# pd3/bcftools

Measured on AMD Instinct MI355X. Metric: variant sites/sec (mpileup|call -m), 1000-sample 30x WGS synthetic, higher is better.
Workload: dtype u8/i32 + f64 likelihood sums

## Files before the change

bcftools_amd/csrc/glfgen.hip:

```cpp
#include <hip/hip_runtime.h>
#include <cstdlib>
#include "kernels.h"

namespace bcfgpu {

#define WG 256
#ifndef GLF_WAVES
#define GLF_WAVES 5
#endif
#define DEF_MAPQ 20
#define CAP_DIST 25

#define NT16_INT_TBL 0x4444444344424104ull
__device__ __forceinline__ int nt16_int(int c) { return (int)((NT16_INT_TBL >> (4 * (c & 15))) & 7); }
__device__ __forceinline__ int tri(int j, int k) { return k * (k + 1) / 2 + j; }

__device__ __forceinline__ uint32_t wave_sum_u32(uint32_t v)
{
    #pragma unroll
    for (int o = 32; o > 0; o >>= 1) v += __shfl_xor(v, o);
    return v;
}

#define LDS_FK   0
#define LDS_CNT  2112
#ifndef NRANK
#define NRANK 10
#endif
#define NSLOT    NRANK
#ifndef FU
#define FU       4
#endif
#define LDS_HIST_OFF (LDS_CNT + NSLOT * WG * 4)
#define HP_SIZE 280
#define HP_MQS  220
#define NPART 17
static_assert(NPART == SITE_NSUM + 3, "phase A's partial sums: the site totals and three mapQ >= 59 counts");

#define KEY_PACK(rev, q, b, sc) ((uint32_t)(rev) | (uint32_t)(q) << 1 | (uint32_t)(b) << 7 | (uint32_t)(sc) << 10)
#define KEY_REV(k)  ((k) & 1u)
#define KEY_Q(k)    (((k) >> 1) & 63u)
#define KEY_B(k)    (((k) >> 7) & 7u)
#define KEY_SC(k)   (((k) >> 10) & 1u)
#define KEY_PRIM    0x800u

#ifndef WR
#define WR 2
#endif
struct PrimSrc {
    const uint16_t *kpp;
    __device__ __forceinline__ uint32_t key(int j) const { return kpp[j]; }
    __device__ __forceinline__ bool ok(uint32_t k) const { return k != 0; }
    __device__ __forceinline__ int operator()(int j) const { const uint32_t k = key(j); return ok(k) ? (int)(k & 0x7f) : -1; }
};
struct BaseSrc {
    const uint16_t *kp; int b;
    __device__ __forceinline__ uint32_t key(int i) const { return kp[i]; }
    __device__ __forceinline__ bool ok(uint32_t k) const { return KEY_B(k) == (uint32_t)b; }
    __device__ __forceinline__ int operator()(int i) const { const uint32_t k = key(i); return ok(k) ? (int)(k & 0x7f) : -1; }
};
__device__ __forceinline__ uint32_t popc64(uint64_t x) { return (uint32_t)__popc((uint32_t)x) + (uint32_t)__popc((uint32_t)(x >> 32)); }
template <bool FIRST, bool CHK, class Src>
__device__ __forceinline__ void count_keys(uint32_t *s_slot, uint64_t qm, int tid, Src src, int nsrc)
{
    const uint64_t qm1 = qm >> 1;
    for (int j = 0; __any(j < nsrc); j += FU) {
        if (j < nsrc) {
            uint32_t k4[FU];
            #pragma unroll
            for (int u = 0; u < FU; ++u) k4[u] = src.key(j + u);
            #pragma unroll
            for (int u = 0; u < FU; ++u) {
                const uint32_t k = k4[u], q = KEY_Q(k);
                const uint32_t r = popc64(qm1 >> q);
                bool take = src.ok(k) && (u == 0 || j + u < nsrc);
                if (!FIRST) take = take && ((qm >> q) & 1ull);
                if (CHK) take = take && r < (uint32_t)NRANK;
                const uint32_t rv = (uint32_t)((int32_t)(k << 31) >> 31);
                if (take) atomicAdd(&s_slot[r * WG + tid], (rv & 1u) | (~rv & 0x100u));
            }
        }
    }
}
template <bool FIRST, class Src>
__device__ __forceinline__ uint32_t count_runs(uint32_t *s_slot, uint64_t qm, int tid, Src src, int nsrc)
{
    #pragma unroll
    for (int k = 0; k < NRANK; ++k) s_slot[k * WG + tid] = 0;
    if (__any(popc64(qm) > (uint32_t)NRANK)) count_keys<FIRST, true>(s_slot, qm, tid, src, nsrc);
    else count_keys<FIRST, false>(s_slot, qm, tid, src, nsrc);
    uint32_t qs = 0;
    uint64_t m = qm;
    #pragma unroll
    for (int r = 0; r < NRANK && __any(m != 0); ++r) {
        if (m != 0) {
            const uint32_t q = 63u - (uint32_t)__builtin_clzll(m);
            const uint32_t c = s_slot[r * WG + tid];
            s_slot[r * WG + tid] = c | q << 16;
            qs = __builtin_amdgcn_udot4(c, q | q << 8, qs, false);
            m &= ~(1ull << q);
        }
    }
    return qs;
}

template <class Src>
__device__ __forceinline__ double walk_runs(uint32_t *s_slot, uint64_t qm, const double *s_fk, const char *bbase, int tid,
                                            uint32_t brow, Src src, int nsrc, uint32_t &rev_out, uint32_t &qs_out)
{
    double bs = 0;
    uint32_t qs = 0;
    uint32_t wpack = 0;
    uint32_t cnt = 0;
    uint32_t koff = brow;
    uint32_t qoff = 0;
    uint32_t r = 0;
    uint32_t d_nx = 0;
    auto slot_of = [&](uint32_t rk) -> uint32_t { return s_slot[min(rk, (uint32_t)NRANK - 1u) * WG + tid]; };
    auto step = [&](uint32_t (&off)[WR], uint32_t (&wi)[WR]) -> bool {
        const bool pop = cnt == 0 && r < NRANK;
        cnt = pop ? (d_nx & 0xffu) | (d_nx & 0xff00u) << 8 : cnt;
        qoff = pop ? (d_nx & 0x3f0000u) << 3 : qoff;
        r += pop ? 1u : 0u;
        d_nx = slot_of(r);
        const uint32_t sh = (cnt & 0xffffu) ? 0u : 16u;
        const uint32_t left = (cnt >> sh) & 0xffffu;
        const uint32_t w = (wpack >> sh) & 0xffffu;
        const uint32_t o1 = qoff + koff;
        #pragma unroll
        for (uint32_t u = 0; u < WR; ++u) {
            const bool act = left > u;
            wi[u] = act ? w + u : 256u;
            off[u] = act ? o1 + (u << 11) : brow;
        }
        const uint32_t took = min(left, (uint32_t)WR);
        wpack += took << sh; cnt -= took << sh;
        koff += took << 11;
        return __any(left != 0);
    };
    #define WALK_LOAD(B, F, off_, wi_) do { _Pragma("unroll") for (int u_ = 0; u_ < WR; ++u_) { \
        B[u_] = *reinterpret_cast<const double*>(bbase + (off_)[u_]); F[u_] = s_fk[(wi_)[u_]]; } } while (0)
    #define WALK_ADD(B, F) do { _Pragma("unroll") for (int u_ = 0; u_ < WR; ++u_) bs += F[u_] * B[u_]; } while (0)
    bool first = true;
    while (__any(qm != 0)) {
        qs += first ? count_runs<true>(s_slot, qm, tid, src, nsrc) : count_runs<false>(s_slot, qm, tid, src, nsrc);
        first = false; r = 0;
        d_nx = slot_of(0);
        double bx[WR], fx[WR], by[WR], fy[WR];
        uint32_t off[WR], wi[WR];
        bool ax = step(off, wi);
        WALK_LOAD(bx, fx, off, wi);
        bool ay = step(off, wi);
        WALK_LOAD(by, fy, off, wi);
        while (ax) {
            WALK_ADD(bx, fx);
            ax = step(off, wi);
            WALK_LOAD(bx, fx, off, wi);
            if (!ay) break;
            WALK_ADD(by, fy);
            ay = step(off, wi);
            WALK_LOAD(by, fy, off, wi);
        }
        WALK_ADD(bx, fx);
        WALK_ADD(by, fy);
        if (__any(__popcll(qm) > NRANK)) {
            uint64_t m = qm;
            for (int k = 0; k < NRANK && m; ++k) m &= ~(1ull << (63 - __clzll((long long)m)));
            qm = m;
        } else qm = 0;
    }
    #undef WALK_ADD
    #undef WALK_LOAD
    rev_out = wpack & 0xffffu; qs_out = qs;
    return bs;
}

struct ReadSums {
    uint32_t t_bq, t_bq2, t_mq, t_mq2, t_md, t_md2;
    uint32_t d_bq, d_bq2, d_mq, d_mq2, d_md, d_md2;
    __device__ __forceinline__ void clear() { t_bq = t_bq2 = t_mq = t_mq2 = t_md = t_md2 = d_bq = d_bq2 = d_mq = d_mq2 = d_md = d_md2 = 0; }
};
struct ReadCounts {
    uint32_t ori, mq0, m59, ref59, rev59;
    __device__ __forceinline__ void clear() { ori = mq0 = m59 = ref59 = rev59 = 0; }
};
typedef unsigned short v2u16 __attribute__((ext_vector_type(2)));

__device__ __forceinline__ uint32_t perm(uint32_t hi, uint32_t lo, uint32_t sel) { return __builtin_amdgcn_perm(hi, lo, sel); }
#define SEL_EVEN 0x0c020c00u
#define SEL_ODD  0x0c030c01u
#define SEL_JOIN 0x06020400u
#define SEL_GE8  0x07030501u
__device__ __forceinline__ v2u16 as_v2(uint32_t x) { return __builtin_bit_cast(v2u16, x); }
__device__ __forceinline__ uint32_t as_u(v2u16 x) { return __builtin_bit_cast(uint32_t, x); }
__device__ __forceinline__ uint32_t pk_min(uint32_t a, uint32_t b) { return as_u(__builtin_elementwise_min(as_v2(a), as_v2(b))); }
__device__ __forceinline__ uint32_t pk_max(uint32_t a, uint32_t b) { return as_u(__builtin_elementwise_max(as_v2(a), as_v2(b))); }
__device__ __forceinline__ uint32_t nonzero80(uint32_t x) { return (((x & 0x7f7f7f7fu) + 0x7f7f7f7fu) | x) & 0x80808080u; }
__device__ __forceinline__ uint32_t bytes_of80(uint32_t m) { return m | (m - (m >> 7)); }
__device__ __forceinline__ uint32_t byte_at(uint32_t x, int u) { return (x >> (8 * u)) & 0xffu; }

template <bool INDEL, bool LDS_HIST, bool DEEP>
__global__ __launch_bounds__(WG) __attribute__((amdgpu_waves_per_eu(GLF_WAVES, GLF_WAVES))) void glfgen_kernel(const GlfgenParams P)
{
    extern __shared__ __align__(16) unsigned char smem[];
    if (DEEP && (blockIdx.x >= P.deep_ctr[0] || P.deep_list[2 * blockIdx.x] == 0xffffffffu)) return;
    const int cap = DEEP ? 0x7ffffff0 : P.lds_cap;
    double   *s_fk  = reinterpret_cast<double*>(smem + LDS_FK);
    uint32_t *s_cnt = reinterpret_cast<uint32_t*>(smem + LDS_CNT);
    int      *s_hist = reinterpret_cast<int*>(smem + LDS_HIST_OFF);
    unsigned long long *s_tot = reinterpret_cast<unsigned long long*>(s_hist + (size_t)P.hist_slots * HP_SIZE);
    uint32_t *s_part = s_cnt;
    const int pcol = P.part_cols;
    uint16_t *s_key = DEEP ? P.deep_keys + P.deep_list[2 * blockIdx.x + 1]
                           : reinterpret_cast<uint16_t*>(s_tot + (size_t)P.hist_slots * SITE_NSUM);
    __shared__ unsigned int s_next, s_skip;

    const int tid = threadIdx.x;
    const int S = P.n_smpl;
    const long ncells = (long)P.n_sites * S;
    const long cell0 = DEEP ? (long)P.deep_list[2 * blockIdx.x] : (long)blockIdx.x * WG;
    const long cell_end = DEEP ? cell0 + 1 : min(cell0 + WG, ncells);
    const int site0 = (int)(cell0 / S);
    const int site_last = (int)((cell_end - 1) / S);

    const long cell = cell0 + tid;
    const bool active = cell < cell_end;

    s_fk[tid] = P.fk[tid];
    if (tid < 8) s_fk[256 + tid] = 0.0;
    if (LDS_HIST) {
        for (int i = tid; i < P.hist_slots * HP_SIZE; i += WG) s_hist[i] = 0;
        for (int i = tid; i < P.hist_slots * SITE_NSUM; i += WG) s_tot[i] = 0;
    }

    int site = 0, ref4c = 4;
    uint32_t beg = 0, end = 0;
    if (active) {
        site = (int)(cell / S);
        beg = P.off[cell]; end = P.off[cell + 1];
        if (!INDEL) ref4c = nt16_int(P.ref16[site]);
    }
    const int primary = INDEL ? 0 : ref4c;
    uint32_t fmt_flag = (uint32_t)P.fmt_flag;
    asm volatile("" : "+s"(fmt_flag));
    const bool want_epos = (fmt_flag & (BCFGPU_INFO_RPB | BCFGPU_INFO_VDB)) != 0;
    const bool want_scr = (fmt_flag & (BCFGPU_INFO_SCR | BCFGPU_FMT_SCR)) != 0;
    const uint32_t span_end = P.off[cell_end];
    uint32_t n_reads_tot = P.n_reads, min_baseQ = (uint32_t)P.min_baseQ, capQ = (uint32_t)P.capQ;
    asm volatile("" : "+s"(n_reads_tot), "+s"(min_baseQ), "+s"(capQ));
    const uint32_t *p_rd = P.rd, *p_aux = P.aux, *p_off = P.off;
    const uint8_t *p_epos = P.epos;
    asm volatile("" : "+s"(p_rd), "+s"(p_aux), "+s"(p_off), "+s"(p_epos));

    bool done = !active;
    bool deep = false;
    if (!DEEP && active && end - beg > (uint32_t)cap - 3u) {
        deep = true;
        const uint32_t need = (end - beg + 16u) & ~7u;
        const uint32_t slot = atomicAdd(&P.deep_ctr[0], 1u), at = atomicAdd(&P.deep_ctr[1], need);
        const bool room = at + need <= P.deep_key_cap;
        if (slot < P.deep_cap) { P.deep_list[2 * slot] = room ? (uint32_t)cell : 0xffffffffu; P.deep_list[2 * slot + 1] = room ? at : 0u; }
        if (slot >= P.deep_cap || !room) { atomicExch(P.err, BCFGPU_E_DEPTH); atomicExch(&P.deep_ctr[2], 1u); }
    }
    uint32_t base = p_off[cell0];

    for (;;) {
        const uint32_t abase = base & ~3u;
        const uint32_t lim = DEEP ? span_end : min(abase + (uint32_t)cap, span_end);
        if (tid == 0) { s_next = 0xffffffffu; s_skip = 0; }
        if (LDS_HIST) {
            int i0 = tid;
            asm volatile("" : "+v"(i0));
            for (int i = i0; i < P.hist_slots * NPART * pcol; i += WG) s_part[i] = 0;
        }
        __syncthreads();
        const bool cand = !done && !deep && beg >= base && end <= lim;
        if (!done && !cand) atomicMin(&s_next, beg);
        __syncthreads();
        const uint32_t nb = s_next;
        const uint32_t rlim = min(nb, lim);
        const bool part = cand && end <= rlim;

        for (int sg = site0; sg <= site_last; ++sg) {
            const long c_lo = max(cell0, (long)sg * S), c_hi = min(cell_end, (long)(sg + 1) * S);
            const uint32_t rb = max(p_off[c_lo], base), re = min(p_off[c_hi], rlim);
            if (rb >= re) continue;
            const int ref_base = INDEL ? -1 : (int)P.ref16[sg];
            const uint32_t ref4 = INDEL ? 4u : (uint32_t)nt16_int(ref_base);
            const uint32_t primq = INDEL ? 0u : ref4;
            const unsigned long long tbl = (NT16_INT_TBL & ~0xfull) | (unsigned long long)ref4;
            int *hist = LDS_HIST ? s_hist + (sg - site0) * HP_SIZE : P.hist + (long)sg * H_SIZE;
            ReadSums A; A.clear();
            ReadCounts C; C.clear();
            const uint32_t tlo_lo = 0x04010000u | ref4, tlo_hi = 0x04040402u, thi_lo = 0x04040403u, thi_hi = 0x04040404u;
            const uint32_t kq = 0x01000100u - min(min_baseQ, 256u) * 0x00010001u;
            const uint32_t cap2 = min(capQ, 0xffffu) * 0x00010001u;
            const uint32_t refb4 = (uint32_t)(ref_base & 15) * 0x01010101u, prim4 = primq * 0x01010101u;
            const uint32_t scm = want_scr ? 0x04040404u : 0u;
            const bool all_diff = !INDEL && ref4 >= 4;
            const bool no_ref = INDEL || ref_base < 0 || ref_base > 15;

            auto quad = [&](const uint4 &w4, const uint4 &a4, uint32_t e4, uint32_t vm4, uint32_t &k01, uint32_t &k23) {
                const uint32_t t0 = perm(w4.y, w4.x, 0x05010400u), t1 = perm(w4.y, w4.x, 0x07030602u);
                const uint32_t t2 = perm(w4.w, w4.z, 0x05010400u), t3 = perm(w4.w, w4.z, 0x07030602u);
                uint32_t B4 = perm(t2, t0, 0x05040100u);
                const uint32_t M4 = perm(t2, t0, 0x07060302u);
                const uint32_t F4 = (vm4 & perm(t3, t1, 0x05040100u)) | (~vm4 & 0x80808080u);
                const uint32_t D4 = perm(t3, t1, 0x07060302u);
                uint32_t QR4, BB4;
                uint32_t ok80;
                const uint32_t seen80 = (INDEL ? F4 : F4 | F4 << 1) & 0x80808080u ^ 0x80808080u;
                if (INDEL) {
                    uint32_t qv[4], bv[4];
                    const uint32_t av[4] = { a4.x, a4.y, a4.z, a4.w }, wv[4] = { w4.x, w4.y, w4.z, w4.w };
                    #pragma unroll
                    for (int u = 0; u < 4; ++u) {
                        const uint32_t ax = av[u];
                        uint32_t b = (ax >> 16) & 0xf, q = ax & 0xff;
                        if (q < min_baseQ) { b = 0; q = wv[u] & 0xff; }
                        bv[u] = min(b, 4u);
                        qv[u] = min(q, (ax >> 8) & 0xff);
                    }
                    B4 = perm(perm(a4.w, a4.z, 0x04000c0cu), perm(a4.y, a4.x, 0x0c0c0400u), 0x07060100u);
                    QR4 = qv[0] | qv[1] << 8 | qv[2] << 16 | qv[3] << 24;
                    BB4 = bv[0] | bv[1] << 8 | bv[2] << 16 | bv[3] << 24;
                    ok80 = seen80;
                } else {
                    const uint32_t ge = perm(perm(0, B4, SEL_ODD) + kq, perm(0, B4, SEL_EVEN) + kq, SEL_GE8);
                    ok80 = seen80 & ge << 7;
                    QR4 = B4;
                    const uint32_t s = F4 & 0x07070707u;
                    BB4 = perm(perm(thi_hi, thi_lo, s), perm(tlo_hi, tlo_lo, s), 0x03020100u | (F4 >> 1 & 0x04040404u));
                }
                const uint32_t OK4 = bytes_of80(ok80);
                const uint32_t me = perm(0, M4, SEL_EVEN), mo = perm(0, M4, SEL_ODD);
                const uint32_t mfe = pk_min(me + (uint32_t)__mul24((int)perm(0, me + 0x00010001u, SEL_ODD), DEF_MAPQ - 255), cap2);
                const uint32_t mfo = pk_min(mo + (uint32_t)__mul24((int)perm(0, mo + 0x00010001u, SEL_ODD), DEF_MAPQ - 255), cap2);
                const uint32_t qe = pk_max(pk_min(pk_min(perm(0, QR4, SEL_EVEN), mfe), 0x003f003fu), 0x00040004u);
                const uint32_t qo = pk_max(pk_min(pk_min(perm(0, QR4, SEL_ODD), mfo), 0x003f003fu), 0x00040004u);
                const uint32_t Q4 = perm(qo, qe, SEL_JOIN);
                const uint32_t Mf4 = perm(mfo, mfe, SEL_JOIN);
                const uint32_t Df4 = perm(pk_min(perm(0, D4, SEL_ODD), 0x00190019u), pk_min(perm(0, D4, SEL_EVEN), 0x00190019u), SEL_JOIN);
                const uint32_t m59_80 = ok80 & perm(mfo + 0x00c500c5u, mfe + 0x00c500c5u, SEL_GE8) << 7;
                const uint32_t nref80 = no_ref ? 0x80808080u : nonzero80((F4 ^ refb4) & 0x0f0f0f0fu);
                C.ori += __builtin_popcount(seen80);
                C.mq0 += __builtin_popcount(ok80 & ~nonzero80(M4));
                C.m59 += __builtin_popcount(m59_80);
                C.ref59 += __builtin_popcount(m59_80 & ~nref80);
                C.rev59 += __builtin_popcount(m59_80 & F4 << 3);
                const uint32_t nprim80 = nonzero80(BB4 ^ prim4);
                const uint32_t klo = (((F4 >> 4) & 0x01010101u) | Q4 << 1 | (BB4 & 0x01010101u) << 7) & OK4;
                const uint32_t khi = (((BB4 >> 1) & 0x03030303u) | ((F4 >> 3) & scm) | ((nprim80 ^ 0x80808080u) >> 4)) & OK4;
                k01 = perm(khi, klo, 0x05010400u); k23 = perm(khi, klo, 0x07030602u);
                const uint32_t Bm = B4 & OK4, Mm = Mf4 & OK4, Dm = Df4 & OK4;
                A.t_bq = __builtin_amdgcn_udot4(Bm, 0x01010101u, A.t_bq, false); A.t_bq2 = __builtin_amdgcn_udot4(Bm, Bm, A.t_bq2, false);
                A.t_mq = __builtin_amdgcn_udot4(Mm, 0x01010101u, A.t_mq, false); A.t_mq2 = __builtin_amdgcn_udot4(Mm, Mm, A.t_mq2, false);
                A.t_md = __builtin_amdgcn_udot4(Dm, 0x01010101u, A.t_md, false); A.t_md2 = __builtin_amdgcn_udot4(Dm, Dm, A.t_md2, false);
                const uint32_t dif80 = ok80 & (all_diff ? 0x80808080u : nprim80);
                if (dif80) {
                    const uint32_t DM = bytes_of80(dif80);
                    const uint32_t bd = Bm & DM, qd = Mm & DM, dd = Dm & DM;
                    A.d_bq = __builtin_amdgcn_udot4(bd, 0x01010101u, A.d_bq, false); A.d_bq2 = __builtin_amdgcn_udot4(bd, bd, A.d_bq2, false);
                    A.d_mq = __builtin_amdgcn_udot4(qd, 0x01010101u, A.d_mq, false); A.d_mq2 = __builtin_amdgcn_udot4(qd, qd, A.d_mq2, false);
                    A.d_md = __builtin_amdgcn_udot4(dd, 0x01010101u, A.d_md, false); A.d_md2 = __builtin_amdgcn_udot4(dd, dd, A.d_md2, false);
                }
                #pragma unroll
                for (int u = 0; u < 4; ++u) {
                    if (!((ok80 >> (8 * u + 7)) & 1)) continue;
                    const bool isref = !((nref80 >> (8 * u + 7)) & 1), rev = (F4 >> (8 * u + 4)) & 1;
                    const uint32_t bq = byte_at(B4, u), mapQ = byte_at(Mf4, u), pos = byte_at(e4, u);
                    const bool m59 = (m59_80 >> (8 * u + 7)) & 1;
                    if (LDS_HIST) {
                        const int inc = isref ? 1 : 0x10000;
                        atomicAdd(&hist[H_REF_POS + pos], inc);
                        atomicAdd(&hist[H_REF_BQ + min(bq, 59u)], inc);
                        if (!m59) {
                            atomicAdd(&hist[H_REF_MQ + mapQ], inc);
                            atomicAdd(&hist[HP_MQS + mapQ], rev ? 0x10000 : 1);
                        }
                    } else {
                        const uint32_t aoff = isref ? 0u : (uint32_t)H_ALT_OFF;
                        atomicAdd(&hist[aoff + H_REF_POS + pos], 1);
                        atomicAdd(&hist[aoff + H_REF_BQ + min(bq, 59u)], 1);
                        if (!m59) {
                            atomicAdd(&hist[aoff + H_REF_MQ + mapQ], 1);
                            atomicAdd(&hist[(rev ? H_REV_MQS : H_FWD_MQS) + mapQ], 1);
                        }
                    }
                }
            };

            const uint32_t g0 = rb & ~3u;
            uint4 w4n = make_uint4(0, 0, 0, 0), a4n = make_uint4(0, 0, 0, 0);
            uint32_t e4n = 0;
            auto fetch = [&](uint32_t i4) {
                if (i4 >= re) return;
                if (i4 + 3 < n_reads_tot) {
                    w4n = *reinterpret_cast<const uint4*>(p_rd + i4);
                    if (want_epos) e4n = *reinterpret_cast<const uint32_t*>(p_epos + i4);
                    if (INDEL) a4n = *reinterpret_cast<const uint4*>(p_aux + i4);
                } else {
                    uint32_t t4[4] = {0, 0, 0, 0}, x4[4] = {0, 0, 0, 0};
                    e4n = 0;
                    for (int j = 0; j < 4; ++j) if (i4 + j < n_reads_tot) {
                        t4[j] = p_rd[i4 + j];
                        if (want_epos) e4n |= (uint32_t)p_epos[i4 + j] << (8 * j);
                        if (INDEL) x4[j] = p_aux[i4 + j];
                    }
                    w4n = make_uint4(t4[0], t4[1], t4[2], t4[3]); a4n = make_uint4(x4[0], x4[1], x4[2], x4[3]);
                }
            };
            fetch(g0 + 4u * tid);
            for (uint32_t i4 = g0 + 4u * tid; i4 < re; i4 += 4u * WG) {
                const uint4 w4 = w4n, a4 = a4n;
                const uint32_t e4 = e4n;
                fetch(i4 + 4u * WG);
                const uint32_t lo = rb > i4 ? rb - i4 : 0u, hi = min(re - i4, 4u);
                const uint32_t vm4 = (0xffffffffu << (8 * lo)) & (hi == 4u ? 0xffffffffu : ~(0xffffffffu << (8 * hi)));
                uint32_t k01, k23;
                quad(w4, a4, e4, vm4, k01, k23);
                const uint32_t ko = i4 - abase;
                if (vm4 == 0xffffffffu) {
                    *reinterpret_cast<uint2*>(s_key + ko) = make_uint2(k01, k23);
                } else {
                    const uint32_t kv[4] = { k01 & 0xffffu, k01 >> 16, k23 & 0xffffu, k23 >> 16 };
                    #pragma unroll
                    for (int u = 0; u < 4; ++u) if ((vm4 >> (8 * u)) & 1) s_key[ko + u] = (uint16_t)kv[u];
                }
            }
            const uint32_t v[NPART] = { A.t_bq - A.d_bq, A.t_bq2 - A.d_bq2, A.d_bq, A.d_bq2, A.t_mq - A.d_mq, A.t_mq2 - A.d_mq2, A.d_mq, A.d_mq2,
                                        A.t_md - A.d_md, A.t_md2 - A.d_md2, A.d_md, A.d_md2, C.ori, C.mq0, C.m59, C.ref59, C.rev59 };
            if (LDS_HIST) {
                uint32_t *pt = s_part + (sg - site0) * (NPART * pcol) + (tid & (pcol - 1));
                #pragma unroll
                for (int j = 0; j < NPART; ++j) atomicAdd(&pt[j * pcol], v[j]);
            } else {
                unsigned long long *tot = P.site_sums + (size_t)sg * SITE_NSUM;
                uint32_t x[NPART];
                #pragma unroll
                for (int j = 0; j < NPART; ++j) x[j] = wave_sum_u32(v[j]);
                if ((tid & 63) == 0) {
                    #pragma unroll
                    for (int j = 0; j < SITE_NSUM; ++j) if (x[j]) atomicAdd(&tot[j], (unsigned long long)x[j]);
                    const uint32_t m59 = x[SITE_NSUM], ref59 = x[SITE_NSUM + 1], rev59 = x[SITE_NSUM + 2];
                    if (ref59) atomicAdd(&hist[H_REF_MQ + 59], (int)ref59);
                    if (m59 - ref59) atomicAdd(&hist[H_ALT_MQ + 59], (int)(m59 - ref59));
                    if (m59 - rev59) atomicAdd(&hist[H_FWD_MQS + 59], (int)(m59 - rev59));
                    if (rev59) atomicAdd(&hist[H_REV_MQS + 59], (int)rev59);
                }
            }
        }
        __syncthreads();
        if (LDS_HIST) {
            const int nslot = min(P.hist_slots, P.n_sites - site0), q4 = pcol >> 2;
            for (int i = tid; i < nslot * NPART * 4; i += WG) {
                const uint32_t *pt = s_part + (i >> 2) * pcol + (i & 3) * q4;
                unsigned long long x = 0;
                for (int k = 0; k < q4; ++k) x += pt[k];
                x += __shfl_xor(x, 1); x += __shfl_xor(x, 2);
                if ((i & 3) == 0 && x) {
                    const int vi = i >> 2, sl = vi / NPART, j = vi % NPART;
                    if (j < SITE_NSUM) s_tot[sl * SITE_NSUM + j] += x;
                    else {
                        const uint32_t c = (uint32_t)x;
                        int *h = s_hist + sl * HP_SIZE;
                        if (j == SITE_NSUM) { atomicAdd(&h[H_REF_MQ + 59], (int)(c << 16)); atomicAdd(&h[HP_MQS + 59], (int)c); }
                        else if (j == SITE_NSUM + 1) atomicAdd(&h[H_REF_MQ + 59], (int)(c - (c << 16)));
                        else atomicAdd(&h[HP_MQS + 59], (int)((c << 16) - c));
                    }
                }
            }
            __syncthreads();
        }

        uint16_t *kp_w = s_key + (part ? beg - abase : 0);
        const uint16_t *kp = kp_w;
        const int cnt_raw = part ? (int)(end - beg) : 0;
        if (__any(cnt_raw > BCFGPU_MAX_DEPTH)) {
            if (cnt_raw > BCFGPU_MAX_DEPTH) {
                uint32_t nus = 0;
                for (int i = 0; i < cnt_raw; ++i) nus += kp_w[i] != 0 ? 1u : 0u;
                const volatile unsigned long long *t = reinterpret_cast<const volatile unsigned long long*>(P.crp);
                uint64_t *qs64_p = reinterpret_cast<uint64_t*>(t[2]); uint32_t *misc_p = reinterpret_cast<uint32_t*>(t[6]);
                uint32_t mark = 0;
                if (nus > BCFGPU_MAX_DEPTH) {
                    uint32_t qs[4] = {0, 0, 0, 0}, af[4] = {0, 0, 0, 0}, ar[4] = {0, 0, 0, 0}, cn[4] = {0, 0, 0, 0}, sc = 0, acc = 0;
                    const bool all_diff = !INDEL && ref4c >= 4;
                    bool planned = false;
                    if (P.draw_bits) {
                        uint32_t nm = 0;
                        for (int i = 0; i < cnt_raw; ++i) { const uint32_t ri = beg + (uint32_t)i; nm += (kp_w[i] != 0 && ((P.draw_bits[ri >> 5] >> (ri & 31)) & 1u)) ? 1u : 0u; }
                        planned = nm == BCFGPU_MAX_DEPTH;
                    }
                    for (int i = 0; i < cnt_raw; ++i) {
                        const uint32_t k = kp_w[i];
                        if (k == 0) continue;
                        const uint32_t rev = KEY_REV(k), q = KEY_Q(k), b = KEY_B(k);
                        const uint32_t dr = ((all_diff || !(k & KEY_PRIM)) ? 2u : 0u) | rev;
                        #pragma unroll
                        for (uint32_t x = 0; x < 4; ++x) {
                            qs[x] += b == x ? q : 0u;
                            af[x] += (b == x && !rev) ? 1u : 0u; ar[x] += (b == x && rev) ? 1u : 0u;
                            cn[x] += dr == x ? 1u : 0u;
                        }
                        sc += KEY_SC(k);
                        bool stays = ++acc <= BCFGPU_MAX_DEPTH;
                        if (planned) { const uint32_t ri = beg + (uint32_t)i; stays = ((P.draw_bits[ri >> 5] >> (ri & 31)) & 1u) != 0; }
                        if (!stays) kp_w[i] = 0;
                    }
                    const uint32_t slot = atomicAdd(P.wide_ctr, 1u);
                    const uint32_t big = af[0] | af[1] | af[2] | af[3] | ar[0] | ar[1] | ar[2] | ar[3] | cn[0] | cn[1] | cn[2] | cn[3] | sc;
                    if (slot >= P.wide_cap || big > 0xffffu) atomicExch(P.err, BCFGPU_E_DEPTH);
                    else {
                        WideRec *w = reinterpret_cast<WideRec*>(t[7]) + slot;
                        #pragma unroll
                        for (int x = 0; x < 4; ++x) { w->qs[x] = qs[x]; w->ad[x] = af[x] | ar[x] << 16; }
                        w->cnt[0] = cn[0] | cn[1] << 16; w->cnt[1] = cn[2] | cn[3] << 16;
                        w->scr = sc; w->n = nus; w->cell = (uint32_t)cell; w->pad[0] = w->pad[1] = w->pad[2] = 0;
                        qs64_p[cell] = WIDE_QS_MARK | slot;
                        mark = CR_WIDE;
                    }
                    if (!planned) atomicAdd(P.trunc, 1u);
                }
                misc_p[cell] = mark;
            }
        }
        uint32_t scr = 0;
        if (want_scr) for (int i = 0; i < cnt_raw; ++i) scr += KEY_SC((uint32_t)kp[i]);
        uint64_t qmask = 0;
        uint32_t n_prim = 0;
        uint64_t qs64 = 0;
        uint64_t ad64 = 0;
        uint32_t n_b4 = 0;
        uint32_t o_rev = 0, n_other = 0;
        {
            uint32_t k_nx = kp[0];
            for (int i = 0; i < cnt_raw; ++i) {
                const uint32_t k = k_nx;
                k_nx = kp[i + 1];
                const uint32_t pb = k >> 11;
                qmask |= (uint64_t)pb << KEY_Q(k);
                n_prim += pb;
                if (k - 1u < KEY_PRIM - 1u) {
                    const uint32_t t = kp_w[n_other], rev = KEY_REV(k), q = KEY_Q(k), b = KEY_B(k);
                    kp_w[n_other] = (uint16_t)k; kp_w[i] = (uint16_t)t;
                    ++n_other; o_rev += rev;
                    if (b < 4) { qs64 += (uint64_t)q << (16 * b); ad64 += 1ull << (8 * b + 32 * rev); }
                    else ++n_b4;
                }
            }
        }
        const uint32_t n = n_prim + n_other;
        const bool dead_cell = n == 0;
        const char *bbase = reinterpret_cast<const char*>(P.beta);
        const uint32_t brow = n << 3;

        double bsum[5] = {0, 0, 0, 0, 0};
        uint32_t prim_rev = 0, qs_prim = 0;
        {
            const uint16_t *kpp = kp + n_other;
            const PrimSrc psrc{kpp};
            const double bs = walk_runs(s_cnt, qmask, s_fk, bbase, tid, brow, psrc, dead_cell ? 0 : cnt_raw - (int)n_other, prim_rev, qs_prim);
            #pragma unroll
            for (int b = 0; b < 5; ++b) if (b == primary) bsum[b] = bs;
        }
        if (primary < 4) {
            qs64 += (uint64_t)qs_prim << (16 * primary);
            ad64 += (uint64_t)(n_prim - prim_rev) << (8 * primary) | (uint64_t)prim_rev << (8 * primary + 32);
        } else n_b4 += n_prim;
        int c[5];
        #pragma unroll
        for (int b = 0; b < 4; ++b) c[b] = (int)((ad64 >> (8 * b)) & 0xff) + (int)((ad64 >> (8 * b + 32)) & 0xff);
        c[4] = (int)n_b4;
        if (__any(n_other > 0)) {
            #pragma unroll 1
            for (int b = 0; b < 5; ++b) {
                int cb = b == 0 ? c[0] : b == 1 ? c[1] : b == 2 ? c[2] : b == 3 ? c[3] : c[4];
                if (b == primary || dead_cell) cb = 0;
                if (!__any(cb > 0)) continue;
                const BaseSrc src{kp, b};
                const int no = cb > 0 ? (int)n_other : 0;
                double bs;
                if (!__any(cb > 1)) {
                    int key = -1;
                    for (int i = 0; __any(i < no); ++i) { const int k7 = i < no ? src(i) : -1; if (k7 >= 0) key = k7; }
                    const uint32_t off1 = key >= 0 ? ((uint32_t)(key >> 1) << 19) + brow : brow;
                    const double B1 = *reinterpret_cast<const double*>(bbase + off1);
                    const double F1 = key >= 0 ? s_fk[0] : s_fk[256];
                    bs = 0.;
                    bs += F1 * B1;
                } else {
                uint64_t qm = 0;
                for (int i = 0; i < no; ++i) { const int key = src(i); if (key >= 0) qm |= 1ull << (key >> 1); }
                uint32_t r_, q_;
                bs = walk_runs(s_cnt, qm, s_fk, bbase, tid, brow, src, no, r_, q_);
                }
                if (cb > 0) {
                    #pragma unroll
                    for (int bb = 0; bb < 5; ++bb) if (bb == b) bsum[bb] = bs;
                }
            }
        }
        const uint32_t n_rev = prim_rev + o_rev;

        uint32_t code = 0;
        CallretPlanes cr;
        {
            const volatile unsigned long long *t = reinterpret_cast<const volatile unsigned long long*>(P.crp);
            cr.p15 = reinterpret_cast<float*>(t[0]); cr.pa = reinterpret_cast<float*>(t[1]);
            cr.qs64 = reinterpret_cast<uint64_t*>(t[2]); cr.adf = reinterpret_cast<uint32_t*>(t[3]);
            cr.adr = reinterpret_cast<uint32_t*>(t[4]); cr.cnt4 = reinterpret_cast<uint32_t*>(t[5]);
            cr.misc = reinterpret_cast<uint32_t*>(t[6]);
        }
        if (part) {
            const int nbases = (c[0] > 0) + (c[1] > 0) + (c[2] > 0) + (c[3] > 0) + (c[4] > 0);
            if (nbases <= 1) {
                const int b = c[1] > 0 ? 1 : c[2] > 0 ? 2 : c[3] > 0 ? 3 : c[4] > 0 ? 4 : 0;
                double bsb = bsum[0];
                #pragma unroll
                for (int k = 1; k < 5; ++k) if (k == b) bsb = bsum[k];
                float A = n > 0 ? (float)((double)0.0f + bsb) : 0.0f;
                if (A < 0.0f) A = 0.0f;
                cr.pa[cell] = A;
                code = (uint32_t)b;
            } else {
                code = CR_FULL;
                float *p15c = cr.p15 + (size_t)cell * 16;
                #pragma unroll
                for (int j = 0; j < 5; ++j) {
                    float tmp1 = 0.0f; int tmp2 = 0;
                    #pragma unroll
                    for (int k = 0; k < 5; ++k) { if (k == j) continue; tmp1 = (float)((double)tmp1 + bsum[k]); tmp2 += c[k]; }
                    float v = 0.0f;
                    if (n > 0 && tmp2) v = tmp1;
                    if (v < 0.0f) v = 0.0f;
                    p15c[tri(j, j)] = v;
                    #pragma unroll
                    for (int k = j + 1; k < 5; ++k) {
                        const int cjk = c[j] + c[k];
                        float t1 = 0.0f; int t2 = 0;
                        #pragma unroll
                        for (int i = 0; i < 5; ++i) { if (i == j || i == k) continue; t1 = (float)((double)t1 + bsum[i]); t2 += c[i]; }
                        float h = 0.0f;
                        if (n > 0) {
                            const double lh = -4.343 * P.lhet[cjk << 8 | c[k]];
                            h = t2 ? (float)(lh + (double)t1) : (float)lh;
                            if (h < 0.0f) h = 0.0f;
                        }
                        p15c[tri(j, k)] = h;
                    }
                }
            }
        }
        if (part) {
            const bool all_diff = (!INDEL && ref4c >= 4);
            const uint32_t n_fwd = n - n_rev;
            const uint32_t d_rev = all_diff ? n_rev : o_rev, d_fwd = all_diff ? n_fwd : n_other - o_rev;
            const uint32_t cnt4 = (n_fwd - d_fwd) | (n_rev - d_rev) << 8 | d_fwd << 16 | d_rev << 24;
            uint32_t wm = 0;
            if (cnt_raw > BCFGPU_MAX_DEPTH) wm = *reinterpret_cast<volatile uint32_t*>(&cr.misc[cell]) & CR_WIDE;
            if (!wm) cr.qs64[cell] = qs64;
            cr.adf[cell] = (uint32_t)ad64; cr.adr[cell] = (uint32_t)(ad64 >> 32); cr.cnt4[cell] = cnt4;
            cr.misc[cell] = code | wm | (scr & 0xff) << 8;
            done = true;
        }
        if (nb == 0xffffffffu) break;
        base = nb;
        if (!DEEP && !done && deep && beg == base) s_skip = end;
        __syncthreads();
        if (!DEEP) {
            const uint32_t sk = s_skip;
            if (sk) { if (deep && beg == base) done = true; base = sk; }
            __syncthreads();
        }
    }

    if (LDS_HIST) {
        __syncthreads();
        const int nslot = min(P.hist_slots, P.n_sites - site0);
        for (int i = tid; i < nslot * HP_SIZE; i += WG) {
            const uint32_t v = (uint32_t)s_hist[i];
            const int sl = i / HP_SIZE, j = i - sl * HP_SIZE;
            int *g = P.hist + (long)(site0 + sl) * H_SIZE;
            const int lo = j < HP_MQS ? j : H_FWD_MQS + (j - HP_MQS), hi = j < HP_MQS ? j + H_ALT_OFF : H_REV_MQS + (j - HP_MQS);
            if (v & 0xffffu) atomicAdd(&g[lo], (int)(v & 0xffffu));
            if (v >> 16) atomicAdd(&g[hi], (int)(v >> 16));
        }
        for (int i = tid; i < nslot * SITE_NSUM; i += WG) {
            const unsigned long long v = s_tot[i];
            if (v) atomicAdd(&P.site_sums[(size_t)site0 * SITE_NSUM + i], v);
        }
    }
}

size_t glfgen_lds_bytes(int cap, int hist_slots)
{
    return LDS_HIST_OFF + (size_t)hist_slots * (HP_SIZE * sizeof(int) + SITE_NSUM * 8) + ((size_t)cap + 8) * 2;
}

template <bool INDEL, bool LDS_HIST>
static void launch_one(const GlfgenParams &p, hipStream_t s, int grid, size_t lds)
{
    if (lds > 48 * 1024)
        hipFuncSetAttribute(reinterpret_cast<const void*>(glfgen_kernel<INDEL, LDS_HIST, false>),
                            hipFuncAttributeMaxDynamicSharedMemorySize, (int)lds);
    hipLaunchKernelGGL((glfgen_kernel<INDEL, LDS_HIST, false>), dim3(grid), dim3(WG), lds, s, p);
    if (p.deep_cap) hipLaunchKernelGGL((glfgen_kernel<INDEL, LDS_HIST, true>), dim3(p.deep_cap), dim3(WG), glfgen_lds_bytes(0, p.hist_slots), s, p);
}

void launch_glfgen(const GlfgenParams &p, hipStream_t s)
{
    const long ncells = (long)p.n_sites * p.n_smpl;
    if (ncells == 0) return;
    const int grid = (int)((ncells + WG - 1) / WG);
    const size_t lds = glfgen_lds_bytes(p.lds_cap, p.hist_slots);
    if (p.is_indel) { if (p.hist_slots) launch_one<true, true>(p, s, grid, lds); else launch_one<true, false>(p, s, grid, lds); }
    else            { if (p.hist_slots) launch_one<false, true>(p, s, grid, lds); else launch_one<false, false>(p, s, grid, lds); }
}

}
```

Before: 6.301 million.

## Issue LDS histogram atomics early with raw LDS addressing and overlap next fetch

The phase-A quad routine now performs the POS and BQ histogram LDS atomics unconditionally per lane, using raw LDS byte addresses computed with SDWA shifts. It issues them before the next global fetch, which is moved inside quad so its loads overlap the rest of the per-quad work. The segment body is templated on a compile-time slot so the first site's histogram base is a constant when LDS starts at address zero. s_next and s_skip are moved into the dynamic LDS region, and several asm barriers steer register and scalar placement. The unconditional atomics add LDS traffic for masked-out lanes that add zero, which is why HP_SIZE must cover any byte index. The lambda duplication also raises code size.

```diff
diff --git a/bcftools_amd/csrc/glfgen.hip b/bcftools_amd/csrc/glfgen.hip
--- a/bcftools_amd/csrc/glfgen.hip
+++ b/bcftools_amd/csrc/glfgen.hip
@@ -1,5 +1,6 @@
 #include <hip/hip_runtime.h>
 #include <cstdlib>
+#include <type_traits>
 #include "kernels.h"
 
 namespace bcfgpu {
@@ -34,6 +35,7 @@
 #define LDS_HIST_OFF (LDS_CNT + NSLOT * WG * 4)
 #define HP_SIZE 280
 #define HP_MQS  220
+static_assert(HP_SIZE >= 256, "a byte is an index into a slot: phase A's POS bin of a read that adds 0 may be any byte");
 #define NPART 17
 static_assert(NPART == SITE_NSUM + 3, "phase A's partial sums: the site totals and three mapQ >= 59 counts");
 
@@ -198,6 +200,18 @@
 __device__ __forceinline__ uint32_t nonzero80(uint32_t x) { return (((x & 0x7f7f7f7fu) + 0x7f7f7f7fu) | x) & 0x80808080u; }
 __device__ __forceinline__ uint32_t bytes_of80(uint32_t m) { return m | (m - (m >> 7)); }
 __device__ __forceinline__ uint32_t byte_at(uint32_t x, int u) { return (x >> (8 * u)) & 0xffu; }
+__device__ __forceinline__ uint32_t byte0_x4(uint32_t x)
+{
+    uint32_t r;
+    asm("v_lshlrev_b32_sdwa %0, %1, %2 dst_sel:DWORD dst_unused:UNUSED_PAD src0_sel:DWORD src1_sel:BYTE_0" : "=v"(r) : "v"(2u), "v"(x));
+    return r;
+}
+typedef __attribute__((address_space(3))) int lds_int;
+__device__ __forceinline__ uint32_t lds_addr(const void *p) { return (uint32_t)(uintptr_t)(const __attribute__((address_space(3))) void*)p; }
+__device__ __forceinline__ void lds_add(uint32_t at, uint32_t v)
+{
+    __hip_atomic_fetch_add(reinterpret_cast<lds_int*>((uintptr_t)at), (int)v, __ATOMIC_RELAXED, __HIP_MEMORY_SCOPE_WORKGROUP);
+}
 
 template <bool INDEL, bool LDS_HIST, bool DEEP>
 __global__ __launch_bounds__(WG) __attribute__((amdgpu_waves_per_eu(GLF_WAVES, GLF_WAVES))) void glfgen_kernel(const GlfgenParams P)
@@ -213,7 +227,8 @@
     const int pcol = P.part_cols;
     uint16_t *s_key = DEEP ? P.deep_keys + P.deep_list[2 * blockIdx.x + 1]
                            : reinterpret_cast<uint16_t*>(s_tot + (size_t)P.hist_slots * SITE_NSUM);
-    __shared__ unsigned int s_next, s_skip;
+    unsigned int &s_next = *reinterpret_cast<unsigned int*>(smem + LDS_FK + 263 * 8), &s_skip = *reinterpret_cast<unsigned int*>(smem + LDS_FK + 263 * 8 + 4);
+    const bool lds0 = lds_addr(smem) == 0;
 
     const int tid = threadIdx.x;
     const int S = P.n_smpl;
@@ -227,7 +242,7 @@
     const bool active = cell < cell_end;
 
     s_fk[tid] = P.fk[tid];
-    if (tid < 8) s_fk[256 + tid] = 0.0;
+    if (tid < 7) s_fk[256 + tid] = 0.0;
     if (LDS_HIST) {
         for (int i = tid; i < P.hist_slots * HP_SIZE; i += WG) s_hist[i] = 0;
         for (int i = tid; i < P.hist_slots * SITE_NSUM; i += WG) s_tot[i] = 0;
@@ -267,7 +282,11 @@
     for (;;) {
         const uint32_t abase = base & ~3u;
         const uint32_t lim = DEEP ? span_end : min(abase + (uint32_t)cap, span_end);
-        if (tid == 0) { s_next = 0xffffffffu; s_skip = 0; }
+        if (tid == 0) {
+            uint32_t none = 0xffffffffu;
+            asm volatile("" : "+v"(none));
+            s_next = none; s_skip = 0;
+        }
         if (LDS_HIST) {
             int i0 = tid;
             asm volatile("" : "+v"(i0));
@@ -285,11 +304,15 @@
             const long c_lo = max(cell0, (long)sg * S), c_hi = min(cell_end, (long)(sg + 1) * S);
             const uint32_t rb = max(p_off[c_lo], base), re = min(p_off[c_hi], rlim);
             if (rb >= re) continue;
+            auto segment = [&](auto slot_c) {
+            constexpr int SLOT = decltype(slot_c)::value;
             const int ref_base = INDEL ? -1 : (int)P.ref16[sg];
             const uint32_t ref4 = INDEL ? 4u : (uint32_t)nt16_int(ref_base);
             const uint32_t primq = INDEL ? 0u : ref4;
             const unsigned long long tbl = (NT16_INT_TBL & ~0xfull) | (unsigned long long)ref4;
-            int *hist = LDS_HIST ? s_hist + (sg - site0) * HP_SIZE : P.hist + (long)sg * H_SIZE;
+            int *hist = P.hist + (long)sg * H_SIZE;
+            const uint32_t hb = SLOT >= 0 ? (uint32_t)(LDS_HIST_OFF + SLOT * HP_SIZE * 4)
+                                          : lds_addr(s_hist) + (uint32_t)(sg - site0) * (HP_SIZE * 4);
             ReadSums A; A.clear();
             ReadCounts C; C.clear();
             const uint32_t tlo_lo = 0x04010000u | ref4, tlo_hi = 0x04040402u, thi_lo = 0x04040403u, thi_hi = 0x04040404u;
@@ -300,9 +323,11 @@
             const bool all_diff = !INDEL && ref4 >= 4;
             const bool no_ref = INDEL || ref_base < 0 || ref_base > 15;
 
-            auto quad = [&](const uint4 &w4, const uint4 &a4, uint32_t e4, uint32_t vm4, uint32_t &k01, uint32_t &k23) {
-                const uint32_t t0 = perm(w4.y, w4.x, 0x05010400u), t1 = perm(w4.y, w4.x, 0x07030602u);
-                const uint32_t t2 = perm(w4.w, w4.z, 0x05010400u), t3 = perm(w4.w, w4.z, 0x07030602u);
+            uint4 w4n = make_uint4(0, 0, 0, 0), a4n = make_uint4(0, 0, 0, 0);
+            uint32_t e4n = 0;
+            auto quad = [&](uint32_t vm4, uint32_t &k01, uint32_t &k23, auto next) {
+                const uint32_t t0 = perm(w4n.y, w4n.x, 0x05010400u), t1 = perm(w4n.y, w4n.x, 0x07030602u);
+                const uint32_t t2 = perm(w4n.w, w4n.z, 0x05010400u), t3 = perm(w4n.w, w4n.z, 0x07030602u);
                 uint32_t B4 = perm(t2, t0, 0x05040100u);
                 const uint32_t M4 = perm(t2, t0, 0x07060302u);
                 const uint32_t F4 = (vm4 & perm(t3, t1, 0x05040100u)) | (~vm4 & 0x80808080u);
@@ -312,12 +337,13 @@
                 const uint32_t seen80 = (INDEL ? F4 : F4 | F4 << 1) & 0x80808080u ^ 0x80808080u;
                 if (INDEL) {
                     uint32_t qv[4], bv[4];
-                    const uint32_t av[4] = { a4.x, a4.y, a4.z, a4.w }, wv[4] = { w4.x, w4.y, w4.z, w4.w };
+                    const uint4 a4 = a4n;
+                    const uint32_t av[4] = { a4.x, a4.y, a4.z, a4.w };
                     #pragma unroll
                     for (int u = 0; u < 4; ++u) {
                         const uint32_t ax = av[u];
                         uint32_t b = (ax >> 16) & 0xf, q = ax & 0xff;
-                        if (q < min_baseQ) { b = 0; q = wv[u] & 0xff; }
+                        if (q < min_baseQ) { b = 0; q = byte_at(B4, u); }
                         bv[u] = min(b, 4u);
                         qv[u] = min(q, (ax >> 8) & 0xff);
                     }
@@ -332,6 +358,20 @@
                     const uint32_t s = F4 & 0x07070707u;
                     BB4 = perm(perm(thi_hi, thi_lo, s), perm(tlo_hi, tlo_lo, s), 0x03020100u | (F4 >> 1 & 0x04040404u));
                 }
+                const uint32_t nref80 = no_ref ? 0x80808080u : nonzero80((F4 ^ refb4) & 0x0f0f0f0fu);
+                uint32_t e4 = 0;
+                if (LDS_HIST) {
+                    const uint32_t alt01 = (ok80 & nref80) >> 7, ref01 = (ok80 >> 7) ^ alt01;
+                    const uint32_t bqe = pk_min(perm(0, B4, SEL_EVEN), 0x003b003bu), bqo = pk_min(perm(0, B4, SEL_ODD), 0x003b003bu);
+                    const uint32_t bq_at[4] = { byte0_x4(bqe), byte0_x4(bqo), bqe >> 16 << 2, bqo >> 16 << 2 };
+                    #pragma unroll
+                    for (int u = 0; u < 4; ++u) {
+                        const uint32_t inc = perm(alt01, ref01, 0x0c040c00u + 0x00010001u * u);
+                        lds_add(hb + 4 * H_REF_POS + (u ? byte_at(e4n, u) << 2 : byte0_x4(e4n)), inc);
+                        lds_add(hb + 4 * H_REF_BQ + bq_at[u], inc);
+                    }
+                } else e4 = e4n;
+                next();
                 const uint32_t OK4 = bytes_of80(ok80);
                 const uint32_t me = perm(0, M4, SEL_EVEN), mo = perm(0, M4, SEL_ODD);
                 const uint32_t mfe = pk_min(me + (uint32_t)__mul24((int)perm(0, me + 0x00010001u, SEL_ODD), DEF_MAPQ - 255), cap2);
@@ -342,7 +382,6 @@
                 const uint32_t Mf4 = perm(mfo, mfe, SEL_JOIN);
                 const uint32_t Df4 = perm(pk_min(perm(0, D4, SEL_ODD), 0x00190019u), pk_min(perm(0, D4, SEL_EVEN), 0x00190019u), SEL_JOIN);
                 const uint32_t m59_80 = ok80 & perm(mfo + 0x00c500c5u, mfe + 0x00c500c5u, SEL_GE8) << 7;
-                const uint32_t nref80 = no_ref ? 0x80808080u : nonzero80((F4 ^ refb4) & 0x0f0f0f0fu);
                 C.ori += __builtin_popcount(seen80);
                 C.mq0 += __builtin_popcount(ok80 & ~nonzero80(M4));
                 C.m59 += __builtin_popcount(m59_80);
@@ -364,25 +403,27 @@
                     A.d_mq = __builtin_amdgcn_udot4(qd, 0x01010101u, A.d_mq, false); A.d_mq2 = __builtin_amdgcn_udot4(qd, qd, A.d_mq2, false);
                     A.d_md = __builtin_amdgcn_udot4(dd, 0x01010101u, A.d_md, false); A.d_md2 = __builtin_amdgcn_udot4(dd, dd, A.d_md2, false);
                 }
-                #pragma unroll
-                for (int u = 0; u < 4; ++u) {
-                    if (!((ok80 >> (8 * u + 7)) & 1)) continue;
-                    const bool isref = !((nref80 >> (8 * u + 7)) & 1), rev = (F4 >> (8 * u + 4)) & 1;
-                    const uint32_t bq = byte_at(B4, u), mapQ = byte_at(Mf4, u), pos = byte_at(e4, u);
-                    const bool m59 = (m59_80 >> (8 * u + 7)) & 1;
-                    if (LDS_HIST) {
-                        const int inc = isref ? 1 : 0x10000;
-                        atomicAdd(&hist[H_REF_POS + pos], inc);
-                        atomicAdd(&hist[H_REF_BQ + min(bq, 59u)], inc);
-                        if (!m59) {
-                            atomicAdd(&hist[H_REF_MQ + mapQ], inc);
-                            atomicAdd(&hist[HP_MQS + mapQ], rev ? 0x10000 : 1);
-                        }
-                    } else {
+                if (LDS_HIST) {
+                    const uint32_t low80 = ok80 & ~m59_80;
+                    const uint32_t alt1 = nref80 >> 7, ref1 = alt1 ^ 0x01010101u;
+                    const uint32_t rev1 = (F4 >> 4) & 0x01010101u, fwd1 = rev1 ^ 0x01010101u;
+                    #pragma unroll
+                    for (int u = 0; u < 4; ++u) {
+                        if (!byte_at(low80, u)) continue;
+                        const uint32_t at = byte_at(Mf4, u) << 2, sel = 0x0c040c00u + 0x00010001u * u;
+                        lds_add(hb + 4 * H_REF_MQ + at, perm(alt1, ref1, sel));
+                        lds_add(hb + 4 * HP_MQS + at, perm(rev1, fwd1, sel));
+                    }
+                } else {
+                    #pragma unroll
+                    for (int u = 0; u < 4; ++u) {
+                        if (!((ok80 >> (8 * u + 7)) & 1)) continue;
+                        const bool isref = !((nref80 >> (8 * u + 7)) & 1), rev = (F4 >> (8 * u + 4)) & 1;
+                        const uint32_t bq = byte_at(B4, u), mapQ = byte_at(Mf4, u), pos = byte_at(e4, u);
                         const uint32_t aoff = isref ? 0u : (uint32_t)H_ALT_OFF;
                         atomicAdd(&hist[aoff + H_REF_POS + pos], 1);
                         atomicAdd(&hist[aoff + H_REF_BQ + min(bq, 59u)], 1);
-                        if (!m59) {
+                        if (!((m59_80 >> (8 * u + 7)) & 1)) {
                             atomicAdd(&hist[aoff + H_REF_MQ + mapQ], 1);
                             atomicAdd(&hist[(rev ? H_REV_MQS : H_FWD_MQS) + mapQ], 1);
                         }
@@ -391,8 +432,6 @@
             };
 
             const uint32_t g0 = rb & ~3u;
-            uint4 w4n = make_uint4(0, 0, 0, 0), a4n = make_uint4(0, 0, 0, 0);
-            uint32_t e4n = 0;
             auto fetch = [&](uint32_t i4) {
                 if (i4 >= re) return;
                 if (i4 + 3 < n_reads_tot) {
@@ -412,13 +451,10 @@
             };
             fetch(g0 + 4u * tid);
             for (uint32_t i4 = g0 + 4u * tid; i4 < re; i4 += 4u * WG) {
-                const uint4 w4 = w4n, a4 = a4n;
-                const uint32_t e4 = e4n;
-                fetch(i4 + 4u * WG);
                 const uint32_t lo = rb > i4 ? rb - i4 : 0u, hi = min(re - i4, 4u);
                 const uint32_t vm4 = (0xffffffffu << (8 * lo)) & (hi == 4u ? 0xffffffffu : ~(0xffffffffu << (8 * hi)));
                 uint32_t k01, k23;
-                quad(w4, a4, e4, vm4, k01, k23);
+                quad(vm4, k01, k23, [&] { fetch(i4 + 4u * WG); });
                 const uint32_t ko = i4 - abase;
                 if (vm4 == 0xffffffffu) {
                     *reinterpret_cast<uint2*>(s_key + ko) = make_uint2(k01, k23);
@@ -449,11 +485,16 @@
                     if (rev59) atomicAdd(&hist[H_REV_MQS + 59], (int)rev59);
                 }
             }
+            };
+            if (!INDEL && !DEEP && LDS_HIST && P.hist_slots == 2 && lds0 && sg == site0) segment(std::integral_constant<int, 0>());
+            else segment(std::integral_constant<int, -1>());
         }
         __syncthreads();
         if (LDS_HIST) {
             const int nslot = min(P.hist_slots, P.n_sites - site0), q4 = pcol >> 2;
-            for (int i = tid; i < nslot * NPART * 4; i += WG) {
+            int i0 = tid;
+            asm volatile("" : "+v"(i0));
+            for (int i = i0; i < nslot * NPART * 4; i += WG) {
                 const uint32_t *pt = s_part + (i >> 2) * pcol + (i & 3) * q4;
                 unsigned long long x = 0;
                 for (int k = 0; k < q4; ++k) x += pt[k];
@@ -517,7 +558,9 @@
                         for (int x = 0; x < 4; ++x) { w->qs[x] = qs[x]; w->ad[x] = af[x] | ar[x] << 16; }
                         w->cnt[0] = cn[0] | cn[1] << 16; w->cnt[1] = cn[2] | cn[3] << 16;
                         w->scr = sc; w->n = nus; w->cell = (uint32_t)cell; w->pad[0] = w->pad[1] = w->pad[2] = 0;
-                        qs64_p[cell] = WIDE_QS_MARK | slot;
+                        uint32_t wm_hi;
+                        asm volatile("v_mov_b32 %0, %1" : "=v"(wm_hi) : "i"((uint32_t)(WIDE_QS_MARK >> 32)));
+                        qs64_p[cell] = (uint64_t)wm_hi << 32 | slot;
                         mark = CR_WIDE;
                     }
                     if (!planned) atomicAdd(P.trunc, 1u);
@@ -565,8 +608,10 @@
             for (int b = 0; b < 5; ++b) if (b == primary) bsum[b] = bs;
         }
         if (primary < 4) {
-            qs64 += (uint64_t)qs_prim << (16 * primary);
-            ad64 += (uint64_t)(n_prim - prim_rev) << (8 * primary) | (uint64_t)prim_rev << (8 * primary + 32);
+            int pb = primary;
+            asm volatile("" : "+v"(pb));
+            qs64 += (uint64_t)qs_prim << (16 * pb);
+            ad64 += (uint64_t)(n_prim - prim_rev) << (8 * pb) | (uint64_t)prim_rev << (8 * pb + 32);
         } else n_b4 += n_prim;
         int c[5];
         #pragma unroll
```

Result: no change. 6.240 million (-1.0%).
